# slatedb/slatedb

Hardware: AMD Instinct MI355X
Metric: GiB/s device-resident SST block encode+bloom, 64 MiB sorted KV, 1/2/4/8 GPU (higher is better)
Workload: dtype u8

## Files before the change

### slatedb_amd/csrc/sdb_encode.h

```cpp
#pragma once
#include <hip/hip_runtime.h>
#include <stdint.h>

#include "../../include/slatedb_amd.h"

namespace sdb {

constexpr uint32_t kChunk = 2048;
constexpr uint32_t kResolveLds = 96 * 1024;
#ifndef SDB_EMIT_CRC_MFMA
#define SDB_EMIT_CRC_SLICE
#endif
#ifdef SDB_EMIT_CRC_SLICE
constexpr uint32_t kCrcLds = 36 * 1024;
#else
constexpr uint32_t kCrcLds = 56 * 1024;
#endif
constexpr uint32_t kImgCap = 4096 + 64;
constexpr uint32_t kStageCap = 4096;
constexpr uint32_t kStageGuard = 64;
constexpr uint32_t kKeyStageCap = 1024;
constexpr uint32_t kPieceRowMax = 4000, kPieceKeyMax = 960, kPieceValMax = 3968;
constexpr uint32_t kSegLook = 1024;
constexpr uint32_t kSegSpan = kChunk + kSegLook;
// ... 58 lines not shown
    uint32_t *lcp;
    uint32_t *szr, *sznr;
    uint64_t *hd;
    uint32_t nfacts;
    uint32_t *row_scratch;
    uint32_t *next;
    uint32_t *bbytes;
    uint32_t *tab_exit;
    uint32_t *tab_cnt;
    uint64_t *tab_bytes;
    uint32_t *anchor_e;
    uint32_t *anchor_blk;
    uint64_t *anchor_byte;
    unsigned long long *err;
    uint32_t *wmax;
    uint32_t *slow_count;
    uint32_t *slow_list;
    uint32_t *big_count;
    uint32_t *big_list;
    BlockDesc *desc;
    uint64_t *stat_part;
    uint32_t *huge_part;
    uint32_t *wmax_part;
    unsigned long long *err_part;
    uint32_t *gtab_exit;
    uint32_t *gtab_cnt;
    uint64_t *gtab_bytes;
    uint32_t *mode;
    uint32_t group;
    uint32_t bloom_fused;
    BloomPlan bpl;
    BloomSlots bq;
    uint8_t *bloom_out;
    uint32_t *done;
    uint32_t nprep_wg;
    uint32_t seg_lds;
    uint8_t *out_data;
    uint64_t *out_block_off;
    uint32_t *out_block_first;
    uint32_t *out_index_key_len;
    uint16_t *out_block_stats;
    uint64_t data_cap, block_cap;
    sdb_sst_summary *summary;
    uint64_t bloom_len;
    uint32_t num_probes, filter_built;
    const uint64_t *bloom_len_dev;
};

struct EncodeWorkspace {
    uint64_t lcp, szr, sznr, hd, row_scratch, next, bbytes, tab_exit, tab_cnt, tab_bytes;
    uint64_t anchor_e, anchor_blk, anchor_byte, err, wmax, slow_count, slow_list, big_count, big_list, desc, stat_part,
        huge_part, wmax_part,
        bloom_rep;
    uint64_t err_part, done, gtab_exit, gtab_cnt, gtab_bytes, mode, blen;
    uint64_t total;
};
uint64_t bloom_workspace_bytes(uint64_t n, uint32_t k, uint64_t bitmap_bytes);
uint64_t encode_bloom_workspace_bytes(uint64_t n, uint32_t k, uint64_t bitmap_bytes);
__host__ __device__ inline EncodeWorkspace encode_workspace_offsets(uint64_t n, bool has_filter) {
    EncodeWorkspace w{};
    uint64_t off = 0;
    auto take = [&](uint64_t bytes) {
        uint64_t r = off;
        off += (bytes + 255) & ~255ull;
        return r;
    };
    uint64_t nc = (n + kChunk - 1) / kChunk;
    w.lcp = take(4 * (n + 1));
    w.szr = take(4 * (n + 1));
    w.sznr = take(4 * (n + 1));
    w.hd = take(0);
    (void)has_filter;
    w.row_scratch = take(4 * (n + 1));
    w.next = take(4 * (n + 1));
    w.bbytes = take(4 * (n + 1));
    w.tab_exit = take(4 * (nc * kSegLook + 1));
    w.tab_cnt = take(4 * (nc * kSegLook + 1));
    w.tab_bytes = take(8 * (nc * kSegLook + 1));
    w.anchor_e = take(4 * (nc + 2));
    w.anchor_blk = take(4 * (nc + 2));
    w.anchor_byte = take(8 * (nc + 2));
    w.err = take(8);
    w.wmax = take(4);
    w.slow_count = take(4);
    w.slow_list = take(4 * (n + 1));
    w.big_count = take(4);
    w.big_list = take(4 * (n + 1));
    w.desc = take(sizeof(BlockDesc) * (n + 1));
    const uint64_t nf = (n + kFactsEntries - 1) / kFactsEntries;
    w.stat_part = take(8 * 5 * (nf + 1));
    w.huge_part = take(4 * (nf + 1));
    w.wmax_part = take(4 * (nc + 1));
    w.err_part = take(8 * (nf + 1));
    w.done = take(8);
    w.gtab_exit = take(4 * (nc * kSegLook + 1));
    w.gtab_cnt = take(4 * (nc * kSegLook + 1));
    w.gtab_bytes = take(8 * (nc * kSegLook + 1));
    w.mode = take(4);
    w.blen = take(8);
    w.bloom_rep = off;
    w.total = off;
    return w;
}
inline EncodeWorkspace encode_workspace_layout(uint64_t n, uint64_t filter_bytes, uint32_t num_probes) {
    EncodeWorkspace w = encode_workspace_offsets(n, filter_bytes != 0);
    w.total = w.bloom_rep + ((filter_bytes ? encode_bloom_workspace_bytes(n, num_probes, filter_bytes) : 0) + 255) / 256 * 256;
    return w;
}
uint64_t prefix_workspace_bytes(uint64_t n);
hipError_t launch_bloom_prefix(const uint8_t *key_bytes, const uint64_t *key_off, const int32_t *lens, uint64_t n,
                               uint32_t bpk, uint32_t kind, uint32_t arg, uint32_t whole, uint8_t *bitmap, uint64_t cap,
                               uint64_t *bloom_len, void *ws, hipStream_t st);
hipError_t launch_bloom_match(const uint8_t *bitmap, uint64_t bytes, uint32_t k, uint32_t whole, uint32_t kind,
                              uint32_t arg, const uint8_t *key_bytes, const uint64_t *key_off, const uint8_t *is_prefix,
                              const int32_t *qlens, uint64_t n, uint8_t *result, hipStream_t st);

constexpr uint32_t kMaxSsts = 8;
enum WsField {
    kWsLcp = 0, kWsSzr, kWsSznr, kWsHd, kWsRowScratch, kWsNext, kWsBbytes, kWsTabExit, kWsTabCnt, kWsTabBytes,
    kWsAnchorE, kWsAnchorBlk, kWsAnchorByte, kWsErr, kWsWmax, kWsSlowCount, kWsSlowList, kWsBigCount, kWsBigList,
    kWsDesc, kWsStatPart, kWsHugePart, kWsWmaxPart, kWsBloomRep, kWsErrPart, kWsDone, kWsGtabExit, kWsGtabCnt,
    kWsGtabBytes, kWsMode, kWsBlen, kWsFields
};
struct SstSlot {
    const uint8_t *key_bytes;
    const uint64_t *key_off;
    const uint8_t *val_bytes;
    const uint64_t *val_off;
    const uint8_t *kind;
    const uint64_t *seq;
    const int64_t *create_ts;
    const int64_t *expire_ts;
    const uint8_t *ts_mask;
    uint64_t n;
    uint8_t *out_data;
    uint64_t *out_block_off;
    uint32_t *out_block_first;
    uint32_t *out_index_key_len;
    uint16_t *out_block_stats;
    uint64_t data_cap, block_cap;
    sdb_sst_summary *summary;
    uint8_t *bloom_out;
    uint64_t bloom_len;
    uint8_t *ws;
    uint32_t num_probes, filter_built, bloom_fused, has_filter_ws;
    uint32_t nchunks, nfacts, group, slot_cap;
    uint32_t prefix_bloom, pad2;
    BloomPlan bpl;
    uint32_t wso[kWsFields];
};
struct SstSet {
    uint32_t count;
    uint32_t block_size, restart_interval, version, wal, seg_look;
    uint32_t max_facts, max_chunks, max_groups, max_tiles, max_slices, pad;
    SstSlot s[kMaxSsts];
};

__host__ __device__ inline EncodeArgs make_args(const SstSet &P, uint32_t i) {
    const SstSlot &s = P.s[i];
    EncodeArgs a{};
    a.key_bytes = s.key_bytes;
    a.key_off = s.key_off;
    a.val_bytes = s.val_bytes;
    a.val_off = s.val_off;
    a.kind = s.kind;
    a.seq = s.seq;
    a.create_ts = s.create_ts;
    a.expire_ts = s.expire_ts;
    a.ts_mask = s.ts_mask;
    a.n = s.n;
    a.block_size = P.block_size;
    a.restart_interval = P.restart_interval;
    a.version = P.version;
    a.wal = P.wal;
    a.nchunks = s.nchunks;
    a.seg_look = P.seg_look;
    uint8_t *b = s.ws;
    auto W = [&](int f) { return b + ((uint64_t)s.wso[f] << 8); };
    a.lcp = (uint32_t *)W(kWsLcp);
    a.szr = (uint32_t *)W(kWsSzr);
    a.sznr = (uint32_t *)W(kWsSznr);
    a.hd = (uint64_t *)W(kWsHd);
    a.nfacts = s.nfacts;
    a.row_scratch = (uint32_t *)W(kWsRowScratch);
    a.next = (uint32_t *)W(kWsNext);
    a.bbytes = (uint32_t *)W(kWsBbytes);
    a.tab_exit = (uint32_t *)W(kWsTabExit);
    a.tab_cnt = (uint32_t *)W(kWsTabCnt);
    a.tab_bytes = (uint64_t *)W(kWsTabBytes);
    a.anchor_e = (uint32_t *)W(kWsAnchorE);
    a.anchor_blk = (uint32_t *)W(kWsAnchorBlk);
    a.anchor_byte = (uint64_t *)W(kWsAnchorByte);
    a.err = (unsigned long long *)W(kWsErr);
    a.wmax = (uint32_t *)W(kWsWmax);
    a.slow_count = (uint32_t *)W(kWsSlowCount);
    a.slow_list = (uint32_t *)W(kWsSlowList);
    a.big_count = (uint32_t *)W(kWsBigCount);
    a.big_list = (uint32_t *)W(kWsBigList);
    a.desc = (BlockDesc *)W(kWsDesc);
    a.stat_part = (uint64_t *)W(kWsStatPart);
    a.huge_part = (uint32_t *)W(kWsHugePart);
    a.wmax_part = (uint32_t *)W(kWsWmaxPart);
    a.err_part = (unsigned long long *)W(kWsErrPart);
    a.gtab_exit = (uint32_t *)W(kWsGtabExit);
    a.gtab_cnt = (uint32_t *)W(kWsGtabCnt);
    a.gtab_bytes = (uint64_t *)W(kWsGtabBytes);
    a.mode = (uint32_t *)W(kWsMode);
    a.group = s.group;
    a.bloom_fused = s.bloom_fused;
    a.bpl = s.bpl;
    {
        uint8_t *q = W(kWsBloomRep);
        a.bq.count = (uint32_t *)q;
        a.bq.slot = (uint32_t *)(q + (((uint64_t)s.bpl.tiles * s.bpl.nslices * 4 + 255) & ~255ull));
        a.bq.cap = s.slot_cap;
    }
    a.bloom_out = s.bloom_out;
    a.done = (uint32_t *)W(kWsDone);
    a.nprep_wg = s.nchunks;
    a.seg_lds = kSegLds;
    a.out_data = s.out_data;
    a.out_block_off = s.out_block_off;
    a.out_block_first = s.out_block_first;
    a.out_index_key_len = s.out_index_key_len;
    a.out_block_stats = s.out_block_stats;
    a.data_cap = s.data_cap;
    a.block_cap = s.block_cap;
    a.summary = s.summary;
    a.bloom_len = s.bloom_len;
    a.num_probes = s.num_probes;
    a.filter_built = s.filter_built;
    a.bloom_len_dev = s.prefix_bloom ? (uint64_t *)W(kWsBlen) : nullptr;
    return a;
}

inline void fill_ws_layout(SstSlot &s) {
    const EncodeWorkspace w = encode_workspace_offsets(s.n, s.has_filter_ws != 0);
    const uint64_t off[kWsFields] = {w.lcp, w.szr, w.sznr, w.hd, w.row_scratch, w.next, w.bbytes, w.tab_exit, w.tab_cnt,
                                     w.tab_bytes, w.anchor_e, w.anchor_blk, w.anchor_byte, w.err, w.wmax, w.slow_count,
                                     w.slow_list, w.big_count, w.big_list, w.desc, w.stat_part, w.huge_part, w.wmax_part,
                                     w.bloom_rep, w.err_part, w.done, w.gtab_exit, w.gtab_cnt, w.gtab_bytes, w.mode, w.blen};
    for (int f = 0; f < kWsFields; f++) s.wso[f] = (uint32_t)(off[f] >> 8);
}

hipError_t launch_encode_set(const SstSet &P, size_t bin_lds, size_t fill_lds, hipStream_t st);
hipError_t launch_encode_empty(EncodeArgs a, hipStream_t st);
hipError_t launch_encode_prep(const SstSet &P, hipStream_t st);

enum Stage { kStBloom = 0, kStFacts, kStSeg, kStAnchor, kStBlocks, kStEmit, kStEmitBig, kStBloomFill, kNumStages };
void stage_mark(hipStream_t st, int stage, bool begin);
bool stage_timing_on();


BloomPlan bloom_plan(uint64_t n, uint32_t k, uint64_t bitmap_bytes, uint32_t tile_keys = 0);
uint64_t bloom_workspace_bytes(uint64_t n, uint32_t k, uint64_t bitmap_bytes);
hipError_t launch_bloom_build(const uint8_t *key_bytes, const uint64_t *key_off, uint64_t n,
                              uint32_t num_probes, uint8_t *bitmap, uint64_t bitmap_bytes, void *ws,
                              hipStream_t st);
hipError_t launch_bloom_query(const uint8_t *bitmap, uint64_t bitmap_bytes, uint32_t num_probes,
                              const uint8_t *key_bytes, const uint64_t *key_off, uint64_t n,
                              uint8_t *result, hipStream_t st);

}
static_assert(sdb::kSegSpan % sdb::kSegThreads == 0 && sdb::kChunk % 64 == 0, "k_seg geometry");
static_assert(sdb::kEmitLds <= 160 * 1024, "k_emit LDS");
static_assert(sizeof(sdb::SstSet) <= 4096, "SstSet is passed as kernel arguments");
```

### slatedb_amd/csrc/sdb_encode.hip

```cpp
#include <stdlib.h>

#include <atomic>
#include <mutex>

#include "sdb_bloom.h"
#include "sdb_crc.h"
#include "sdb_crc_mfma.h"

namespace sdb {

#ifndef SDB_SEG_WAVES
#define SDB_SEG_WAVES 8
#endif
#ifdef SDB_PHASE_TIMING
__device__ uint64_t g_phase[1024][8];
#define PHASE_MARK(i)                                                              \
    do {                                                                           \
        __syncthreads();                                                           \
        if (threadIdx.x == 0 && blockIdx.x < 1024) g_phase[blockIdx.x][i] = __builtin_amdgcn_s_memtime(); \
    } while (0)
__device__ uint64_t g_wave_phase[8192][8];
__device__ uint64_t g_phase_enum[1024][8];
#define PHASE_MARK_E(i)                                                                  \
    do {                                                                                 \
        __syncthreads();                                                                 \
        if (threadIdx.x == 0 && blockIdx.x < 1024) g_phase_enum[blockIdx.x][i] = __builtin_amdgcn_s_memtime(); \
    } while (0)
__device__ uint64_t g_wave_rt[8192][4];
#define WAVE_T(var)                                     \
    uint64_t var = __builtin_amdgcn_s_memtime();        \
    __builtin_amdgcn_s_waitcnt(0xC07F)
#define PHASE_MARK_AT(slot, i)                                                        \
    do {                                                                          \
        __syncthreads();                                                          \
        if (threadIdx.x == 0) g_phase[slot][i] = __builtin_amdgcn_s_memtime();   \
    } while (0)
#else
#define PHASE_MARK(i) \
    do {              \
    } while (0)
#define PHASE_MARK_AT(slot, i) \
    do {                       \
    } while (0)
#define PHASE_MARK_E(i) \
    do {                \
    } while (0)
#define WAVE_T(var) \
    do {            \
    } while (0)
#endif


struct EntryFacts {
    uint32_t lcp, s_r, s_nr;
    uint64_t klen, vlen;
    uint8_t kind;
    int err;
};

struct FactsIn {
    uint64_t pko, ko0, ko1, vo0, vo1;
    uint64_t pk0, pk1, ck0, ck1;
    uint8_t kd, m;
};

SDB_DEV void facts_load_offsets(const EncodeArgs &a, uint64_t i, FactsIn &in) {
    in.ko0 = a.key_off[i];
    in.ko1 = a.key_off[i + 1];
    in.pko = i > 0 ? a.key_off[i - 1] : in.ko0;
    in.vo0 = a.val_off[i];
    in.vo1 = a.val_off[i + 1];
    in.kd = a.kind ? a.kind[i] : 0;
    in.m = a.ts_mask ? a.ts_mask[i] : 0;
}

SDB_DEV void facts_load_keys(const EncodeArgs &a, FactsIn &in) {
    const uint64_t klen = in.ko1 - in.ko0, plen = in.ko0 - in.pko;
    uint64_t n = klen < plen ? klen : plen;
    n = n < 16 ? n : 16;
    in.pk0 = in.ck0 = in.pk1 = in.ck1 = 0;
    if (n) {
        const uint32_t n0 = (uint32_t)(n < 8 ? n : 8);
        in.pk0 = load8(a.key_bytes + in.pko, n0);
        in.ck0 = load8(a.key_bytes + in.ko0, n0);
        if (n > 8) {
            in.pk1 = load8(a.key_bytes + in.pko + 8, (uint32_t)(n - 8));
            in.ck1 = load8(a.key_bytes + in.ko0 + 8, (uint32_t)(n - 8));
        }
    }
}

SDB_DEV EntryFacts facts_finish(const EncodeArgs &a, uint64_t i, const FactsIn &in) {
    EntryFacts f;
    const uint64_t klen = in.ko1 - in.ko0;
    const uint8_t kd = in.kd, m = in.m;
    const uint64_t vlen = (kd == SDB_KIND_TOMBSTONE) ? 0 : (in.vo1 - in.vo0);
    uint32_t lcp = 0;
    int err = 0;
    if (kd > SDB_KIND_TOMBSTONE) err = SDB_INVALID_ARGUMENT;
    if (!err && i > 0) {
        const uint64_t plen = in.ko0 - in.pko;
        const uint64_t mn = plen < klen ? plen : klen;
        const uint32_t nmin = (uint32_t)(mn > 0xFFFFFFFFull ? 0xFFFFFFFFull : mn);
        const uint32_t n0 = nmin < 8 ? nmin : 8, n1 = nmin < 16 ? nmin - n0 : 8;
        uint64_t x0 = in.pk0 ^ in.ck0, x1 = in.pk1 ^ in.ck1;
        if (n0 < 8) x0 &= (1ull << (8 * n0)) - 1;
        if (n1 < 8) x1 &= (1ull << (8 * n1)) - 1;
        if (x0) lcp = __builtin_ctzll(x0) >> 3;
        else if (x1) lcp = 8 + (__builtin_ctzll(x1) >> 3);
        else if (nmin <= 16) lcp = nmin;
        else lcp = 16 + lcp_bytes(a.key_bytes + in.pko + 16, nmin - 16, a.key_bytes + in.ko0 + 16, nmin - 16);
        if (klen == 0) err = SDB_EMPTY_KEY;
        else if (!a.wal && plen > 0 && lcp == klen && klen < plen) err = SDB_INVALID_ARGUMENT;
    }
    if (!err && klen == 0) err = SDB_EMPTY_KEY;
    const uint32_t ts8 = 8u * (((m & SDB_TS_CREATE) != 0) + ((m & SDB_TS_EXPIRE) != 0));
    if (a.version == 2) {
        if (!err && (klen > 0xFFFFFFFFull || vlen > 0xFFFFFFFFull)) err = SDB_LIMIT_EXCEEDED;
        uint32_t kl = (uint32_t)klen, vl = (uint32_t)vlen, suf = kl - lcp;
        f.s_nr = varint_len(lcp) + varint_len(suf) + varint_len(vl) + suf + vl + 9 + ts8;
        f.s_r = 1 + varint_len(kl) + varint_len(vl) + kl + vl + 9 + ts8;
    } else {
        if (!err && (klen > 0xFFFF || vlen > 0xFFFFFFFFull)) err = SDB_LIMIT_EXCEEDED;
        f.s_r = (uint32_t)(4 + klen + 9 + ts8 + (kd == SDB_KIND_TOMBSTONE ? 0 : 4 + vlen));
        f.s_nr = f.s_r;
    }
    f.lcp = lcp;
    f.klen = klen;
    f.vlen = vlen;
    f.kind = kd;
    f.err = err;
    return f;
}

SDB_DEV EntryFacts entry_facts(const EncodeArgs &a, uint64_t i) {
    FactsIn in;
    facts_load_offsets(a, i, in);
    facts_load_keys(a, in);
    return facts_finish(a, i, in);
}

__global__ __launch_bounds__(kFactsThreads, 8) void k_facts(SstSet P) {
    const EncodeArgs a = make_args(P, blockIdx.y);
    if (blockIdx.x >= a.nfacts) return;
    extern __shared__ __attribute__((aligned(16))) uint32_t blds[];
    __shared__ uint64_t s_part[kFactsThreads / 64][5];
    __shared__ unsigned long long s_err[kFactsThreads / 64];
    __shared__ uint32_t s_huge[kFactsThreads / 64];
    const uint32_t tid = threadIdx.x, lane = (uint32_t)lane_id();
    const uint64_t e0 = (uint64_t)blockIdx.x * kFactsEntries + tid;
    const uint64_t n = a.n;
    FactsIn in[kFactsPerT];
#pragma unroll
    for (uint32_t r = 0; r < kFactsPerT; r++) {
        const uint64_t e = e0 + r * kFactsThreads;
        FactsIn &f = in[r];
        f.ko0 = f.ko1 = f.vo0 = f.vo1 = f.pko = 0;
        f.kd = f.m = 0;
        if (e <= n) {
            f.ko0 = a.key_off[e];
            f.vo0 = a.val_off[e];
            if (e < n) {
                f.kd = a.kind ? a.kind[e] : 0;
                f.m = a.ts_mask ? a.ts_mask[e] : 0;
                if (lane == 63) {
                    f.ko1 = a.key_off[e + 1];
                    f.vo1 = a.val_off[e + 1];
                }
                if (lane == 0 && e > 0) f.pko = a.key_off[e - 1];
            }
        }
    }
    const uint64_t ktot = a.key_off[n];
#pragma unroll
    for (uint32_t r = 0; r < kFactsPerT; r++) {
        FactsIn &f = in[r];
        const uint64_t nk = wave_next_lane(f.ko0), nv = wave_next_lane(f.vo0);
        if (lane != 63) {
            f.ko1 = nk;
            f.vo1 = nv;
        }
        const uint64_t e = e0 + r * kFactsThreads;
        const bool live = e < n;
        const uint8_t *safe = (const uint8_t *)a.key_off;
        const uint8_t *cs = live && f.ko0 + 16 <= ktot ? a.key_bytes + f.ko0 : safe;
        uint4 cw;
        __builtin_memcpy(&cw, cs, 16);
        f.ck0 = (uint64_t)cw.x | (uint64_t)cw.y << 32;
        f.ck1 = (uint64_t)cw.z | (uint64_t)cw.w << 32;
        f.pk0 = f.pk1 = 0;
    }
#pragma unroll
    for (uint32_t r = 0; r < kFactsPerT; r++) {
        FactsIn &f = in[r];
        const uint64_t e = e0 + r * kFactsThreads;
        if (lane == 0 && e > 0 && e < n && f.pko + 16 <= ktot) {
            uint4 pw;
            __builtin_memcpy(&pw, a.key_bytes + f.pko, 16);
            f.pk0 = (uint64_t)pw.x | (uint64_t)pw.y << 32;
            f.pk1 = (uint64_t)pw.z | (uint64_t)pw.w << 32;
        }
    }
#pragma unroll
    for (uint32_t r = 0; r < kFactsPerT; r++) {
        FactsIn &f = in[r];
        const uint64_t e = e0 + r * kFactsThreads;
        if (e < n && f.ko0 + 16 > ktot) {
            const uint64_t kl = f.ko1 - f.ko0;
            const uint32_t kn = (uint32_t)(kl < 16 ? kl : 16);
            f.ck0 = f.ck1 = 0;
            if (kn) f.ck0 = load8(a.key_bytes + f.ko0, kn < 8 ? kn : 8);
            if (kn > 8) f.ck1 = load8(a.key_bytes + f.ko0 + 8, kn - 8);
        }
        if (lane == 0 && e > 0 && e < n && f.pko + 16 > ktot) {
            const uint64_t pl = f.ko0 - f.pko;
            const uint32_t pn = (uint32_t)(pl < 16 ? pl : 16);
            f.pk0 = f.pk1 = 0;
            if (pn) f.pk0 = load8(a.key_bytes + f.pko, pn < 8 ? pn : 8);
            if (pn > 8) f.pk1 = load8(a.key_bytes + f.pko + 8, pn - 8);
        }
    }
    uint64_t rk = 0, rv = 0, c = 0;
    uint64_t err = ~0ull;
    bool huge = false;
    uint32_t hh[kFactsPerT], dd[kFactsPerT];
#pragma unroll
    for (uint32_t r = 0; r < kFactsPerT; r++) {
        FactsIn &f = in[r];
        const uint64_t e = e0 + r * kFactsThreads;
        {
            const uint64_t pko = wave_prev_lane(f.ko0), pk0 = wave_prev_lane(f.ck0), pk1 = wave_prev_lane(f.ck1);
            if (lane != 0) {
                f.pko = pko;
                f.pk0 = pk0;
                f.pk1 = pk1;
            } else if (e == 0) {
                f.pko = f.ko0;
            }
        }
        hh[r] = dd[r] = 0;
        if (e < n) {
            const EntryFacts x = facts_finish(a, e, f);
            a.lcp[e] = x.lcp;
            a.szr[e] = x.s_r;
            a.sznr[e] = x.s_nr;
            if (a.bloom_fused) {
                const uint64_t kl = f.ko1 - f.ko0;
#ifdef SDB_EXP_FACTS_NOHASH
                const uint64_t h = (f.ck0 * 0x9E3779B97F4A7C15ull) ^ (f.ck1 + kl);
#else
                const uint64_t h = kl == 16 ? siphash13_16(f.ck0, f.ck1) : siphash13(a.key_bytes + f.ko0, kl);
#endif
                hh[r] = fastmod_u32((uint32_t)h, a.bpl.mmod, a.bpl.m);
                dd[r] = fastmod_u32((uint32_t)(h >> 32), a.bpl.mmod, a.bpl.m);
            }
            if (x.err) {
                const uint64_t ev = (e << 8) | (uint64_t)x.err;
                err = ev < err ? ev : err;
            }
            huge |= x.s_r > kPieceRowMax || x.klen > kPieceKeyMax || x.vlen > kPieceValMax;
            rk += x.klen;
            rv += x.vlen;
            c += (uint64_t)(x.kind == SDB_KIND_VALUE) | ((uint64_t)(x.kind == SDB_KIND_TOMBSTONE) << 20) |
                 ((uint64_t)(x.kind == SDB_KIND_MERGE) << 40);
        }
    }
    rk = wave_sum(rk);
    rv = wave_sum(rv);
    c = wave_sum(c);
    err = wave_readlane(wave_incl_scan_op(err, [](uint64_t x, uint64_t y) { return x < y ? x : y; }), 63);
    const uint32_t w = tid >> 6;
    if (lane == 0) {
        s_part[w][0] = rk;
        s_part[w][1] = rv;
        s_part[w][2] = c & 0xFFFFF;
        s_part[w][3] = (c >> 20) & 0xFFFFF;
        s_part[w][4] = (c >> 40) & 0xFFFFF;
        s_err[w] = err;
    }
    const bool wh = __ballot(huge) != 0;
    if (lane == 0) s_huge[w] = wh ? 1u : 0u;
    __syncthreads();
    if (tid < 5) {
        uint64_t t = 0;
        for (uint32_t q = 0; q < kFactsThreads / 64; q++) t += s_part[q][tid];
        a.stat_part[5 * (uint64_t)blockIdx.x + tid] = t;
    }
    if (tid == 0) {
        unsigned long long m = ~0ull;
        for (uint32_t q = 0; q < kFactsThreads / 64; q++) m = s_err[q] < m ? s_err[q] : m;
        a.err_part[blockIdx.x] = m;
        uint32_t h = 0;
        for (uint32_t q = 0; q < kFactsThreads / 64; q++) h |= s_huge[q];
        a.huge_part[blockIdx.x] = h;
    }
    if (a.bloom_fused) {
        const uint64_t k0 = (uint64_t)blockIdx.x * kFactsEntries;
        const uint32_t nk = (uint32_t)((k0 + kFactsEntries < n ? k0 + kFactsEntries : n) - k0);
#ifdef SDB_EXP_FACTS_NOBIN
        bloom_bin_core<kFactsPerT>(blockIdx.x, hh, dd, 0, a.bpl, a.bq, blds);
#else
        bloom_bin_core<kFactsPerT>(blockIdx.x, hh, dd, nk, a.bpl, a.bq, blds);
#endif
    }
}

SDB_DEV uint32_t walk_size_v2(const EncodeArgs &a, uint64_t j, bool rs) {
    EntryFacts f = entry_facts(a, j);
    return rs ? f.s_r : f.s_nr;
}

SDB_DEV void seg_chunk(const EncodeArgs &a, uint8_t *smem, uint32_t k) {
    uint32_t *s_P = (uint32_t *)smem;
    uint32_t *s_R = s_P + kSegSpan + 4;
    uint32_t *s_bb = s_R + kSegSpan;
    uint16_t *s_nx = (uint16_t *)(s_bb + kChunk);
    __shared__ uint32_t s_len[kSegThreads / 64];
    const uint32_t tid = threadIdx.x, nt = blockDim.x;
    const uint64_t cs = (uint64_t)k * kChunk;
    const uint64_t ce = cs + kChunk < a.n ? cs + kChunk : a.n;
    const uint64_t se = ce + a.seg_look < a.n ? ce + a.seg_look : a.n;
    const uint32_t cn = (uint32_t)(ce - cs), sn = (uint32_t)(se - cs);
    const uint64_t bs = a.block_size;
    const uint32_t clampv = (uint32_t)(bs + 16);
    const bool v2 = a.version == 2 && bs <= (1u << 20);
    const uint32_t ri = a.restart_interval;
    PHASE_MARK(0);
    constexpr uint32_t kPerT = kSegSpan / kSegThreads;
    const uint32_t lane = (uint32_t)lane_id();
    uint32_t zr[kPerT], znr[kPerT];
#pragma unroll
    for (uint32_t u = 0; u < kPerT; u++) {
        const uint32_t x = tid + u * nt;
        zr[u] = znr[u] = 0;
        if (x < sn) {
            zr[u] = a.szr[cs + x];
            znr[u] = a.sznr[cs + x];
        }
    }
#pragma unroll
    for (uint32_t u = 0; u < kPerT; u++) {
        const uint32_t x = tid + u * nt;
        if (x >= sn) continue;
        if (v2) {
            const uint32_t cr = zr[u] < clampv ? zr[u] : clampv, cnr = znr[u] < clampv ? znr[u] : clampv;
            s_P[x] = cnr;
            s_R[x] = cr + 2 - cnr;
        }
    }
    __syncthreads();
    PHASE_MARK(1);
    if (v2) {
        __shared__ uint32_t s_wt[kPerT * (kSegThreads / 64) + 1];
        const uint32_t wv = tid >> 6;
        uint32_t v[kPerT], inc[kPerT];
#pragma unroll
        for (uint32_t u = 0; u < kPerT; u++) {
            const uint32_t x = tid + u * nt;
            v[u] = x < sn ? s_P[x] : 0;
            inc[u] = wave_incl_scan(v[u]);
            if (lane == 63) s_wt[u * (nt >> 6) + wv] = inc[u];
        }
        __syncthreads();
        if (tid < 64) {
            const uint32_t nw = kPerT * (nt >> 6);
            const uint32_t t = tid < nw ? s_wt[tid] : 0, it = wave_incl_scan(t);
            __builtin_amdgcn_wave_barrier();
            if (tid < nw) s_wt[tid] = it - t;
            if (tid == 63) s_P[sn] = it;
        }
        __syncthreads();
#pragma unroll
        for (uint32_t u = 0; u < kPerT; u++) {
            const uint32_t x = tid + u * nt;
            if (x < sn) s_P[x] = s_wt[u * (nt >> 6) + wv] + inc[u] - v[u];
        }
        PHASE_MARK(2);
    }
    __syncthreads();
    PHASE_MARK(3);
    uint32_t maxlen = 0;
    for (uint32_t x = tid; x < cn; x += nt) {
        const uint64_t b = cs + x;
        uint64_t j;
        uint64_t bytes;
        if (v2) {
            const uint32_t Pb = s_P[x];
            auto size_of = [&](uint32_t e) -> uint64_t {
                uint64_t sz = 2ull + (s_P[e] - Pb);
                for (uint32_t r = x; r < e; r += ri) sz += s_R[r];
                return sz;
            };
            uint32_t lo = x + 1;
            uint32_t e = lo;
            {
                const uint32_t w = (x + 64 < sn ? x + 64 : sn) - x;
                const uint32_t mean = (s_P[x + w] - Pb) / w + 1;
                uint32_t est = x + (uint32_t)(bs / mean);
                e = est < lo ? lo : (est > sn ? sn : est);
            }
            if (size_of(e) <= bs) {
                while (e < sn && size_of(e + 1) <= bs) e++;
            } else {
                while (e > lo && size_of(e) > bs) e--;
            }
            j = cs + e;
            if (e == lo) bytes = 2ull + a.szr[b] + 2;
            else bytes = size_of(e);
            if (e == sn && se < a.n) {
                uint64_t acc = bytes;
                uint32_t p = e - x, ph = p % ri;
                while (j < a.n) {
                    const bool rs = ph == 0;
                    const uint64_t add = (uint64_t)walk_size_v2(a, j, rs) + (rs ? 2 : 0);
                    if (acc + add > bs) break;
                    acc += add;
                    j++;
                    if (++ph == ri) ph = 0;
                }
                bytes = acc;
            }
        } else if (a.version == 2) {
            uint64_t acc = 2;
            j = b;
            uint32_t p = 0, ph = 0;
            while (j < a.n) {
                const bool rs = ph == 0;
                const uint64_t add = (uint64_t)walk_size_v2(a, j, rs) + (rs ? 2 : 0);
                if (p > 0 && acc + add > bs) break;
                acc += add;
                j++;
                p++;
                if (++ph == ri) ph = 0;
            }
            bytes = acc;
        } else {
            uint64_t acc = 2;
            j = b;
            uint32_t p = 0;
            const uint64_t fko = a.key_off[b];
            const uint32_t fkl = (uint32_t)(a.key_off[b + 1] - fko);
            while (j < a.n) {
                uint32_t prefix = 0;
                if (p > 0) {
                    uint64_t ko = a.key_off[j];
                    prefix = lcp_bytes(a.key_bytes + fko, fkl, a.key_bytes + ko, (uint32_t)(a.key_off[j + 1] - ko));
                }
                uint64_t sr = a.szr[j];
                uint64_t sz = sr - prefix;
                if (p > 0 && acc + sz > bs) break;
                acc += sz + 2;
                j++;
                p++;
            }
            bytes = acc;
        }
        const uint32_t bb = (uint32_t)(bytes + 4);
// ... 2052 lines not shown
    }
}

template __global__ void k_emit<1>(SstSet);
template __global__ void k_emit<2>(SstSet);

template <int V>
__global__ __launch_bounds__(kEmitThreads, 1) void k_emit_big(SstSet P) {
    extern __shared__ __attribute__((aligned(16))) uint8_t smem[];
    uint32_t pre[kMaxSsts + 1];
    pre[0] = 0;
#pragma unroll
    for (uint32_t i = 0; i < kMaxSsts; i++) {
        uint32_t nb = 0;
        if (i < P.count) {
            const EncodeArgs ai = make_args(P, i);
            if (*ai.err == ~0ull) nb = *ai.big_count;
        }
        pre[i + 1] = pre[i] + nb;
    }
    const uint32_t total = pre[kMaxSsts];
    if (!total || lds_addr((const void *)smem) != 0) return;
    crc_tables_to_lds((lu32 *)smem);
    __syncthreads();
    const uint32_t wave = (uint32_t)__builtin_amdgcn_readfirstlane((int)(threadIdx.x >> 6)), wpb = blockDim.x >> 6;
    lu8 *img = (lu8 *)smem + kCrcLds + 16 + wave * kEmitWaveLds + kStageGuard;
    lu8 *kst = img + kImgCap + 16;
    lSpanCopy *rtab = (lSpanCopy *)(kst + kKeyStageCap);
    for (uint32_t g = blockIdx.x * wpb + wave; g < total; g += gridDim.x * wpb) {
        uint32_t si = 0, base = 0;
#pragma unroll
        for (uint32_t j = 1; j < kMaxSsts; j++)
            if (g >= pre[j] && pre[j] < total) {
                si = j;
                base = pre[j];
            }
        const EncodeArgs a = make_args(P, si);
        const uint32_t blk = a.big_list[g - base];
        emit_big<V>(a, blk, a.desc[blk], img, kst, rtab);
    }
}
template __global__ void k_emit_big<1>(SstSet);
template __global__ void k_emit_big<2>(SstSet);

__global__ void k_init_summary(EncodeArgs a) {
    if (threadIdx.x == 0) {
        sdb_sst_summary *s = a.summary;
        s->data_len = 0;
        s->num_blocks = 0;
        s->num_entries = a.n;
        s->raw_key_size = 0;
        s->raw_val_size = 0;
        s->num_puts = s->num_deletes = s->num_merges = 0;
        s->bloom_len = 0;
        s->num_probes = 0;
        s->filter_built = 0;
        s->status = 0;
        s->max_block_entries = 0;
        s->first_error_entry = ~0ull;
        *a.err = ~0ull;
        *a.wmax = 0;
        *a.slow_count = 0;
        *a.big_count = 0;
        if (a.n == 0 && a.block_cap + 1 > 0) {
            a.out_block_off[0] = 0;
            a.out_block_first[0] = 0;
        }
    }
}

__global__ void k_finish_summary(EncodeArgs a, uint64_t bloom_len, uint32_t num_probes, uint32_t built) {
    if (threadIdx.x == 0) {
        sdb_sst_summary *s = a.summary;
        unsigned long long e = *a.err;
        s->max_block_entries = *a.wmax;
        s->bloom_len = bloom_len;
        s->num_probes = num_probes;
        s->filter_built = built;
        if (e != ~0ull) {
            s->status = (int32_t)(e & 0xFF);
            s->first_error_entry = e >> 8;
        }
    }
}

#ifdef SDB_PHASE_TIMING
extern "C" int sdb_diag_wave_phase(uint64_t *out, int nwaves) {
    return hipMemcpyFromSymbol(out, HIP_SYMBOL(g_wave_phase), sizeof(uint64_t) * 8 * nwaves) == hipSuccess ? 0 : -1;
}
extern "C" int sdb_diag_wave_rt(uint64_t *out, int nwaves) {
#ifdef SDB_PHASE_TIMING
    return hipMemcpyFromSymbol(out, HIP_SYMBOL(g_wave_rt), sizeof(uint64_t) * 4 * nwaves) == hipSuccess ? 0 : -1;
#else
    return -1;
#endif
}
extern "C" int sdb_diag_enum_phase(uint64_t *out, int nblocks) {
    return hipMemcpyFromSymbol(out, HIP_SYMBOL(g_phase_enum), sizeof(uint64_t) * 8 * nblocks) == hipSuccess ? 0 : -1;
}
extern "C" int sdb_diag_phase_times(uint64_t *out, int nblocks) {
    return hipMemcpyFromSymbol(out, HIP_SYMBOL(g_phase), sizeof(uint64_t) * 8 * nblocks) == hipSuccess ? 0 : -1;
}
#endif

static int g_cus = 0;
static uint32_t g_emit_threads = kEmitThreads, g_emit_wg_per_cu = kEmitWgPerCu;
static std::once_flag g_attrs_once;
static uint32_t g_emit_grid = 0;
constexpr int kMaxDevices = 64;
static std::atomic<uint32_t> g_builders[kMaxDevices];
static int current_device() {
    int dev = 0;
    return hipGetDevice(&dev) == hipSuccess && dev >= 0 && dev < kMaxDevices ? dev : 0;
}
static uint32_t emit_grid() {
    if (g_emit_grid) return g_emit_grid;
    const uint32_t full = (uint32_t)(g_cus > 0 ? g_emit_wg_per_cu * g_cus : 512);
    const uint32_t b = g_builders[current_device()].load(std::memory_order_relaxed);
    return b > 1 ? (full / b ? full / b : 1u) : full;
}
static uint32_t emit_lds() { return kCrcLds + 16 + (g_emit_threads / 64) * kEmitWaveLds; }
static void set_lds_attrs() {
    std::call_once(g_attrs_once, [] {
        int dev = 0;
        (void)hipGetDevice(&dev);
        (void)hipDeviceGetAttribute(&g_cus, hipDeviceAttributeMultiprocessorCount, dev);
        if (const char *e = getenv("SDB_EMIT_THREADS")) {
            uint32_t t = (uint32_t)atoi(e);
            if (t >= 64 && t <= kEmitThreads && t % 64 == 0) g_emit_threads = t;
        }
        if (const char *e = getenv("SDB_EMIT_GRID")) {
            const int t = atoi(e);
            if (t >= 1 && t <= 4096) g_emit_grid = (uint32_t)t;
        }
        if (const char *e = getenv("SDB_EMIT_WG_PER_CU")) {
            uint32_t t = (uint32_t)atoi(e);
            if (t >= 1 && t <= 32) g_emit_wg_per_cu = t;
        }
        (void)hipFuncSetAttribute((const void *)k_emit<1>, hipFuncAttributeMaxDynamicSharedMemorySize, (int)kEmitLds);
        (void)hipFuncSetAttribute((const void *)k_emit<2>, hipFuncAttributeMaxDynamicSharedMemorySize, (int)kEmitLds);
        (void)hipFuncSetAttribute((const void *)k_emit_big<1>, hipFuncAttributeMaxDynamicSharedMemorySize, (int)kEmitLds);
        (void)hipFuncSetAttribute((const void *)k_emit_big<2>, hipFuncAttributeMaxDynamicSharedMemorySize, (int)kEmitLds);
        (void)hipFuncSetAttribute((const void *)k_enum, hipFuncAttributeMaxDynamicSharedMemorySize, (int)kEnumLds);
        (void)hipFuncSetAttribute((const void *)k_group, hipFuncAttributeMaxDynamicSharedMemorySize, (int)kGroupLds);
        (void)hipFuncSetAttribute((const void *)k_anchor, hipFuncAttributeMaxDynamicSharedMemorySize, (int)kAnchorLds);
        (void)hipFuncSetAttribute((const void *)k_seg, hipFuncAttributeMaxDynamicSharedMemorySize, 96 * 1024);
        (void)hipFuncSetAttribute((const void *)k_facts, hipFuncAttributeMaxDynamicSharedMemorySize, (int)kBinLds);
        (void)hipGetLastError();
    });
}

static_assert(kChunk == kFactsEntries && kFactsThreads == kBinThreads, "bloom tiles are k_facts' chunks of kChunk keys");

hipError_t launch_encode_set(const SstSet &P, size_t bin_lds, size_t fill_lds, hipStream_t st) {
    set_lds_attrs();
    if (!P.count) return hipSuccess;
    stage_mark(st, kStFacts, true);
    hipLaunchKernelGGL(k_facts, dim3(P.max_facts, P.count), dim3(kFactsThreads), P.max_tiles ? bin_lds : 0, st, P);
    stage_mark(st, kStFacts, false);
    stage_mark(st, kStSeg, true);
    const size_t seg_lds = kSegLds > fill_lds ? kSegLds : fill_lds;
    hipLaunchKernelGGL(k_seg, dim3(P.max_chunks + P.max_slices, P.count), dim3(kSegThreads), seg_lds, st, P);
    stage_mark(st, kStSeg, false);
    stage_mark(st, kStAnchor, true);
    hipLaunchKernelGGL(k_anchor, dim3(1, P.count), dim3(kAnchorThreads), kAnchorLds, st, P);
    stage_mark(st, kStAnchor, false);
    stage_mark(st, kStBlocks, true);
    hipLaunchKernelGGL(k_blocks, dim3(P.max_chunks, P.count), dim3(kBlkThreads), 0, st, P);
    stage_mark(st, kStBlocks, false);
    stage_mark(st, kStEmitBig, true);
    const uint32_t big_grid = P.block_size > 4096 ? emit_grid() : (emit_grid() < 32 ? emit_grid() : 32);
    if (P.version == 2) hipLaunchKernelGGL(k_emit_big<2>, dim3(big_grid), dim3(g_emit_threads), emit_lds(), st, P);
    else hipLaunchKernelGGL(k_emit_big<1>, dim3(big_grid), dim3(g_emit_threads), emit_lds(), st, P);
    stage_mark(st, kStEmitBig, false);
    stage_mark(st, kStEmit, true);
    if (P.version == 2) hipLaunchKernelGGL(k_emit<2>, dim3(emit_grid()), dim3(g_emit_threads), emit_lds(), st, P);
    else hipLaunchKernelGGL(k_emit<1>, dim3(emit_grid()), dim3(g_emit_threads), emit_lds(), st, P);
    stage_mark(st, kStEmit, false);
    return hipGetLastError();
}

hipError_t launch_encode_prep(const SstSet &P, hipStream_t st) {
    set_lds_attrs();
    if (!P.count) return hipSuccess;
    hipLaunchKernelGGL(k_facts, dim3(P.max_facts, P.count), dim3(kFactsThreads), 0, st, P);
    hipLaunchKernelGGL(k_seg, dim3(P.max_chunks, P.count), dim3(kSegThreads), kSegLds, st, P);
    hipLaunchKernelGGL(k_group, dim3(P.max_groups, P.count), dim3(kGroupThreads), kGroupLds, st, P);
    return hipGetLastError();
}

hipError_t launch_encode_empty(EncodeArgs a, hipStream_t st) {
    hipLaunchKernelGGL(k_init_summary, dim3(1), dim3(64), 0, st, a);
    hipLaunchKernelGGL(k_finish_summary, dim3(1), dim3(64), 0, st, a, a.bloom_len, a.num_probes, a.filter_built);
    return hipGetLastError();
}

}

extern "C" sdb_status sdb_set_concurrent_builders(uint32_t builders) {
    if (builders == 0) return SDB_INVALID_ARGUMENT;
    sdb::g_builders[sdb::current_device()].store(builders, std::memory_order_relaxed);
    return SDB_OK;
}
```

Before: 1228.

## Add 32-bit narrow-offset fast path to k_facts tiles

Adds a narrow path in k_facts that, when the key and value byte spans fit in 32 bits, loads only the low halves of the offsets and does all per-entry arithmetic and reductions in 32-bit. It also shares neighbour offsets and the first 16 key bytes across lanes with wave shuffles instead of loading them again from memory. The aim is less ALU, register and load work in the facts stage, with the shared per-tile epilogue moved into a helper. In exchange it keeps two code paths and adds per-block range checks, and the kind-count packing now uses 10-bit fields, which assumes per-wave counts stay below 1024.

```diff
diff --git a/slatedb_amd/csrc/sdb_encode.h b/slatedb_amd/csrc/sdb_encode.h
--- a/slatedb_amd/csrc/sdb_encode.h
+++ b/slatedb_amd/csrc/sdb_encode.h
@@ -234,7 +234,8 @@
 struct SstSet {
     uint32_t count;
     uint32_t block_size, restart_interval, version, wal, seg_look;
-    uint32_t max_facts, max_chunks, max_groups, max_tiles, max_slices, pad;
+    uint32_t max_facts, max_chunks, max_groups, max_tiles, max_slices;
+    uint32_t facts_narrow_limit;
     SstSlot s[kMaxSsts];
 };
 
diff --git a/slatedb_amd/csrc/sdb_encode.hip b/slatedb_amd/csrc/sdb_encode.hip
--- a/slatedb_amd/csrc/sdb_encode.hip
+++ b/slatedb_amd/csrc/sdb_encode.hip
@@ -140,13 +140,293 @@
     return facts_finish(a, i, in);
 }
 
+struct FactsLds {
+    uint64_t part[kFactsThreads / 64][5];
+    unsigned long long err[kFactsThreads / 64];
+    uint32_t huge[kFactsThreads / 64];
+};
+
+SDB_DEV void facts_tile_finish(const EncodeArgs &a, FactsLds &s, const uint32_t (&hh)[kFactsPerT],
+                               const uint32_t (&dd)[kFactsPerT], uint32_t *blds) {
+    const uint32_t tid = threadIdx.x;
+    const uint64_t n = a.n;
+    __syncthreads();
+    if (tid < 5) {
+        uint64_t t = 0;
+        for (uint32_t q = 0; q < kFactsThreads / 64; q++) t += s.part[q][tid];
+        a.stat_part[5 * (uint64_t)blockIdx.x + tid] = t;
+    }
+    if (tid == 0) {
+        unsigned long long m = ~0ull;
+        for (uint32_t q = 0; q < kFactsThreads / 64; q++) m = s.err[q] < m ? s.err[q] : m;
+        a.err_part[blockIdx.x] = m;
+        uint32_t h = 0;
+        for (uint32_t q = 0; q < kFactsThreads / 64; q++) h |= s.huge[q];
+        a.huge_part[blockIdx.x] = h;
+    }
+    if (a.bloom_fused) {
+        const uint64_t k0 = (uint64_t)blockIdx.x * kFactsEntries;
+        const uint32_t nk = (uint32_t)((k0 + kFactsEntries < n ? k0 + kFactsEntries : n) - k0);
+#ifdef SDB_EXP_FACTS_NOBIN
+        bloom_bin_core<kFactsPerT>(blockIdx.x, hh, dd, 0, a.bpl, a.bq, blds);
+#else
+        bloom_bin_core<kFactsPerT>(blockIdx.x, hh, dd, nk, a.bpl, a.bq, blds);
+#endif
+    }
+}
+
+struct FactsIn32 {
+    uint32_t pko, ko0, ko1, vo0, vo1;
+    uint32_t pk[4], ck[4];
+    uint8_t kd, m;
+};
+struct EntryFacts32 {
+    uint32_t lcp, s_r, s_nr, klen, vlen;
+    uint8_t kind;
+    int err;
+};
+
+SDB_DEV EntryFacts32 facts_finish32(const EncodeArgs &a, bool has_prev, const uint8_t *kbase, const FactsIn32 &in) {
+    EntryFacts32 f;
+    const uint32_t klen = in.ko1 - in.ko0;
+    const uint8_t kd = in.kd, m = in.m;
+    const uint32_t vlen = (kd == SDB_KIND_TOMBSTONE) ? 0 : (in.vo1 - in.vo0);
+    uint32_t lcp = 0;
+    int err = 0;
+    if (kd > SDB_KIND_TOMBSTONE) err = SDB_INVALID_ARGUMENT;
+    if (!err && has_prev) {
+        const uint32_t plen = in.ko0 - in.pko;
+        const uint32_t nmin = plen < klen ? plen : klen;
+        const uint64_t x0 = ((uint64_t)(in.pk[1] ^ in.ck[1]) << 32) | (in.pk[0] ^ in.ck[0]);
+        const uint64_t x1 = ((uint64_t)(in.pk[3] ^ in.ck[3]) << 32) | (in.pk[2] ^ in.ck[2]);
+        const uint32_t d = x0 ? (uint32_t)(__builtin_ctzll(x0) >> 3) : x1 ? 8 + (uint32_t)(__builtin_ctzll(x1) >> 3) : 16;
+        if (d < 16 || nmin <= 16) lcp = d < nmin ? d : nmin;
+        else lcp = 16 + lcp_bytes(kbase + in.pko + 16, nmin - 16, kbase + in.ko0 + 16, nmin - 16);
+        if (klen == 0) err = SDB_EMPTY_KEY;
+        else if (!a.wal && plen > 0 && lcp == klen && klen < plen) err = SDB_INVALID_ARGUMENT;
+    }
+    if (!err && klen == 0) err = SDB_EMPTY_KEY;
+    const uint32_t ts8 = 8u * (((m & SDB_TS_CREATE) != 0) + ((m & SDB_TS_EXPIRE) != 0));
+    if (a.version == 2) {
+        const uint32_t suf = klen - lcp;
+        f.s_nr = varint_len(lcp) + varint_len(suf) + varint_len(vlen) + suf + vlen + 9 + ts8;
+        f.s_r = 1 + varint_len(klen) + varint_len(vlen) + klen + vlen + 9 + ts8;
+    } else {
+        if (!err && klen > 0xFFFF) err = SDB_LIMIT_EXCEEDED;
+        f.s_r = 4 + klen + 9 + ts8 + (kd == SDB_KIND_TOMBSTONE ? 0 : 4 + vlen);
+        f.s_nr = f.s_r;
+    }
+    f.lcp = lcp;
+    f.klen = klen;
+    f.vlen = vlen;
+    f.kind = kd;
+    f.err = err;
+    return f;
+}
+
+SDB_DEV uint32_t facts_nrel(const EncodeArgs &a, uint64_t t0) {
+    return (uint32_t)(a.n - t0 < kFactsEntries + 1 ? a.n - t0 : kFactsEntries + 1);
+}
+
+SDB_DEV void facts_narrow_load(const EncodeArgs &a, uint64_t t0, FactsIn32 (&in)[kFactsPerT]) {
+    const uint32_t tid = threadIdx.x, lane = (uint32_t)lane_id();
+    const uint32_t nrel = facts_nrel(a, t0);
+    const bool tile0 = t0 == 0;
+    const uint32_t *kol = (const uint32_t *)(a.key_off + t0), *vol = (const uint32_t *)(a.val_off + t0);
+    const uint8_t *kindb = a.kind ? a.kind + t0 : nullptr, *maskb = a.ts_mask ? a.ts_mask + t0 : nullptr;
+#pragma unroll
+    for (uint32_t r = 0; r < kFactsPerT; r++) {
+        const uint32_t i = tid + r * kFactsThreads;
+        FactsIn32 &f = in[r];
+        f.ko0 = f.ko1 = f.vo0 = f.vo1 = f.pko = 0;
+        f.kd = f.m = 0;
+        if (i <= nrel) {
+            f.ko0 = kol[2 * i];
+            f.vo0 = vol[2 * i];
+            if (i < nrel) {
+                f.kd = kindb ? kindb[i] : 0;
+                f.m = maskb ? maskb[i] : 0;
+                if (lane == 63) {
+                    f.ko1 = kol[2 * i + 2];
+                    f.vo1 = vol[2 * i + 2];
+                }
+                if (lane == 0 && (i > 0 || !tile0)) f.pko = kol[2 * (int32_t)i - 2];
+            }
+        }
+    }
+}
+
+SDB_DEV void facts_tile_narrow(const EncodeArgs &a, uint64_t t0, FactsLds &s, uint32_t (&hh)[kFactsPerT],
+                                  uint32_t (&dd)[kFactsPerT]) {
+    const uint32_t tid = threadIdx.x, lane = (uint32_t)lane_id();
+    const uint32_t nrel = facts_nrel(a, t0);
+    const bool tile0 = t0 == 0;
+    const uint64_t kb = a.key_off[t0 ? t0 - 1 : 0], vb = a.val_off[t0];
+    const uint8_t *kbase = a.key_bytes + kb;
+    const uint32_t kb32 = (uint32_t)kb, vb32 = (uint32_t)vb;
+    FactsIn32 in[kFactsPerT];
+    facts_narrow_load(a, t0, in);
+#pragma unroll
+    for (uint32_t r = 0; r < kFactsPerT; r++) {
+        FactsIn32 &f = in[r];
+        f.ko0 -= kb32;
+        f.ko1 -= kb32;
+        f.pko -= kb32;
+        f.vo0 -= vb32;
+        f.vo1 -= vb32;
+    }
+    const uint64_t ktr = a.key_off[a.n] - kb;
+    const bool anyk = ktr >= 16;
+    const uint32_t klim = (uint32_t)(ktr > 0xFFFFFFFFull ? 0xFFFFFFFFull : ktr) - 16;
+    const uint8_t *wbase = anyk ? kbase : (const uint8_t *)a.key_off;
+#pragma unroll
+    for (uint32_t r = 0; r < kFactsPerT; r++) {
+        FactsIn32 &f = in[r];
+        const uint32_t nk = wave_next_lane(f.ko0), nv = wave_next_lane(f.vo0);
+        if (lane != 63) {
+            f.ko1 = nk;
+            f.vo1 = nv;
+        }
+        const uint32_t i = tid + r * kFactsThreads;
+        const uint32_t wo = i < nrel && anyk && f.ko0 <= klim ? f.ko0 : 0;
+        uint4 cw;
+        __builtin_memcpy(&cw, wbase + wo, 16);
+        f.ck[0] = cw.x;
+        f.ck[1] = cw.y;
+        f.ck[2] = cw.z;
+        f.ck[3] = cw.w;
+        f.pk[0] = f.pk[1] = f.pk[2] = f.pk[3] = 0;
+    }
+#pragma unroll
+    for (uint32_t r = 0; r < kFactsPerT; r++) {
+        FactsIn32 &f = in[r];
+        const uint32_t i = tid + r * kFactsThreads;
+        if (lane == 0 && (i > 0 || !tile0) && i < nrel && anyk && f.pko <= klim) {
+            uint4 pw;
+            __builtin_memcpy(&pw, kbase + f.pko, 16);
+            f.pk[0] = pw.x;
+            f.pk[1] = pw.y;
+            f.pk[2] = pw.z;
+            f.pk[3] = pw.w;
+        }
+    }
+#pragma unroll
+    for (uint32_t r = 0; r < kFactsPerT; r++) {
+        FactsIn32 &f = in[r];
+        const uint32_t i = tid + r * kFactsThreads;
+        if (i < nrel && !(anyk && f.ko0 <= klim)) {
+            const uint32_t kl = f.ko1 - f.ko0;
+            const uint32_t kn = kl < 16 ? kl : 16;
+            uint64_t c0 = 0, c1 = 0;
+            if (kn) c0 = load8(kbase + f.ko0, kn < 8 ? kn : 8);
+            if (kn > 8) c1 = load8(kbase + f.ko0 + 8, kn - 8);
+            f.ck[0] = (uint32_t)c0;
+            f.ck[1] = (uint32_t)(c0 >> 32);
+            f.ck[2] = (uint32_t)c1;
+            f.ck[3] = (uint32_t)(c1 >> 32);
+        }
+        if (lane == 0 && (i > 0 || !tile0) && i < nrel && !(anyk && f.pko <= klim)) {
+            const uint32_t pl = f.ko0 - f.pko;
+            const uint32_t pn = pl < 16 ? pl : 16;
+            uint64_t p0 = 0, p1 = 0;
+            if (pn) p0 = load8(kbase + f.pko, pn < 8 ? pn : 8);
+            if (pn > 8) p1 = load8(kbase + f.pko + 8, pn - 8);
+            f.pk[0] = (uint32_t)p0;
+            f.pk[1] = (uint32_t)(p0 >> 32);
+            f.pk[2] = (uint32_t)p1;
+            f.pk[3] = (uint32_t)(p1 >> 32);
+        }
+    }
+    uint32_t rk = 0, rv = 0, c = 0, nerr = 0;
+    bool huge = false;
+    uint32_t *lcpo = a.lcp + t0, *szro = a.szr + t0, *sznro = a.sznr + t0;
+#pragma unroll
+    for (uint32_t r = 0; r < kFactsPerT; r++) {
+        FactsIn32 &f = in[r];
+        const uint32_t i = tid + r * kFactsThreads;
+        {
+            const uint32_t pko = wave_prev_lane(f.ko0);
+            const uint32_t p0 = wave_prev_lane(f.ck[0]), p1 = wave_prev_lane(f.ck[1]);
+            const uint32_t p2 = wave_prev_lane(f.ck[2]), p3 = wave_prev_lane(f.ck[3]);
+            if (lane != 0) {
+                f.pko = pko;
+                f.pk[0] = p0;
+                f.pk[1] = p1;
+                f.pk[2] = p2;
+                f.pk[3] = p3;
+            } else if (i == 0 && tile0) {
+                f.pko = f.ko0;
+            }
+        }
+        hh[r] = dd[r] = 0;
+        if (i < nrel) {
+            const EntryFacts32 x = facts_finish32(a, i > 0 || !tile0, kbase, f);
+            lcpo[i] = x.lcp;
+            szro[i] = x.s_r;
+            sznro[i] = x.s_nr;
+            if (a.bloom_fused) {
+                const uint64_t ck0 = ((uint64_t)f.ck[1] << 32) | f.ck[0], ck1 = ((uint64_t)f.ck[3] << 32) | f.ck[2];
+#ifdef SDB_EXP_FACTS_NOHASH
+                const uint64_t h = (ck0 * 0x9E3779B97F4A7C15ull) ^ (ck1 + x.klen);
+#else
+                const uint64_t h = x.klen == 16 ? siphash13_16(ck0, ck1) : siphash13(kbase + f.ko0, x.klen);
+#endif
+                hh[r] = fastmod_u32((uint32_t)h, a.bpl.mmod, a.bpl.m);
+                dd[r] = fastmod_u32((uint32_t)(h >> 32), a.bpl.mmod, a.bpl.m);
+            }
+            if (x.err) {
+                const uint32_t ne = ~((i << 8) | (uint32_t)x.err);
+                nerr = ne > nerr ? ne : nerr;
+            }
+            huge |= x.s_r > kPieceRowMax || x.klen > kPieceKeyMax || x.vlen > kPieceValMax;
+            rk += x.klen;
+            rv += x.vlen;
+            c += (uint32_t)(x.kind == SDB_KIND_VALUE) | ((uint32_t)(x.kind == SDB_KIND_TOMBSTONE) << 10) |
+                 ((uint32_t)(x.kind == SDB_KIND_MERGE) << 20);
+        }
+    }
+    rk = wave_sum(rk);
+    rv = wave_sum(rv);
+    c = wave_sum(c);
+    nerr = wave_max(nerr);
+    const uint32_t w = tid >> 6;
+    if (lane == 0) {
+        s.part[w][0] = rk;
+        s.part[w][1] = rv;
+        s.part[w][2] = c & 0x3FF;
+        s.part[w][3] = (c >> 10) & 0x3FF;
+        s.part[w][4] = (c >> 20) & 0x3FF;
+        s.err[w] = nerr ? (t0 << 8) + (uint32_t)~nerr : ~0ull;
+    }
+    const bool wh = __ballot(huge) != 0;
+    if (lane == 0) s.huge[w] = wh ? 1u : 0u;
+}
+
 __global__ __launch_bounds__(kFactsThreads, 8) void k_facts(SstSet P) {
     const EncodeArgs a = make_args(P, blockIdx.y);
     if (blockIdx.x >= a.nfacts) return;
     extern __shared__ __attribute__((aligned(16))) uint32_t blds[];
-    __shared__ uint64_t s_part[kFactsThreads / 64][5];
-    __shared__ unsigned long long s_err[kFactsThreads / 64];
-    __shared__ uint32_t s_huge[kFactsThreads / 64];
+    __shared__ FactsLds s;
+    {
+        const uint64_t t0 = (uint64_t)blockIdx.x * kFactsEntries;
+        const uint64_t lim = P.facts_narrow_limit ? P.facts_narrow_limit : 1ull << 32;
+        const uint64_t kfirst = a.key_off[0], klast = a.key_off[a.n], vfirst = a.val_off[0], vlast = a.val_off[a.n];
+        bool narrow = (klast - kfirst < lim) & (vlast - vfirst < lim);
+        if (!narrow) {
+            const uint64_t t1 = t0 + kFactsEntries < a.n ? t0 + kFactsEntries : a.n;
+            const uint64_t kb = a.key_off[t0 ? t0 - 1 : 0], vb = a.val_off[t0];
+            narrow = (a.key_off[t1] - kb < lim) & (a.val_off[t1] - vb < lim);
+        }
+        if (narrow) {
+            uint32_t sst = blockIdx.y;
+            asm volatile("" : "+s"(sst));
+            uint32_t hh[kFactsPerT], dd[kFactsPerT];
+            facts_tile_narrow(make_args(P, sst), t0, s, hh, dd);
+            asm volatile("" : "+s"(sst));
+            facts_tile_finish(make_args(P, sst), s, hh, dd, blds);
+            return;
+        }
+    }
     const uint32_t tid = threadIdx.x, lane = (uint32_t)lane_id();
     const uint64_t e0 = (uint64_t)blockIdx.x * kFactsEntries + tid;
     const uint64_t n = a.n;
@@ -271,38 +551,16 @@
     err = wave_readlane(wave_incl_scan_op(err, [](uint64_t x, uint64_t y) { return x < y ? x : y; }), 63);
     const uint32_t w = tid >> 6;
     if (lane == 0) {
-        s_part[w][0] = rk;
-        s_part[w][1] = rv;
-        s_part[w][2] = c & 0xFFFFF;
-        s_part[w][3] = (c >> 20) & 0xFFFFF;
-        s_part[w][4] = (c >> 40) & 0xFFFFF;
-        s_err[w] = err;
+        s.part[w][0] = rk;
+        s.part[w][1] = rv;
+        s.part[w][2] = c & 0xFFFFF;
+        s.part[w][3] = (c >> 20) & 0xFFFFF;
+        s.part[w][4] = (c >> 40) & 0xFFFFF;
+        s.err[w] = err;
     }
     const bool wh = __ballot(huge) != 0;
-    if (lane == 0) s_huge[w] = wh ? 1u : 0u;
-    __syncthreads();
-    if (tid < 5) {
-        uint64_t t = 0;
-        for (uint32_t q = 0; q < kFactsThreads / 64; q++) t += s_part[q][tid];
-        a.stat_part[5 * (uint64_t)blockIdx.x + tid] = t;
-    }
-    if (tid == 0) {
-        unsigned long long m = ~0ull;
-        for (uint32_t q = 0; q < kFactsThreads / 64; q++) m = s_err[q] < m ? s_err[q] : m;
-        a.err_part[blockIdx.x] = m;
-        uint32_t h = 0;
-        for (uint32_t q = 0; q < kFactsThreads / 64; q++) h |= s_huge[q];
-        a.huge_part[blockIdx.x] = h;
-    }
-    if (a.bloom_fused) {
-        const uint64_t k0 = (uint64_t)blockIdx.x * kFactsEntries;
-        const uint32_t nk = (uint32_t)((k0 + kFactsEntries < n ? k0 + kFactsEntries : n) - k0);
-#ifdef SDB_EXP_FACTS_NOBIN
-        bloom_bin_core<kFactsPerT>(blockIdx.x, hh, dd, 0, a.bpl, a.bq, blds);
-#else
-        bloom_bin_core<kFactsPerT>(blockIdx.x, hh, dd, nk, a.bpl, a.bq, blds);
-#endif
-    }
+    if (lane == 0) s.huge[w] = wh ? 1u : 0u;
+    facts_tile_finish(a, s, hh, dd, blds);
 }
 
 SDB_DEV uint32_t walk_size_v2(const EncodeArgs &a, uint64_t j, bool rs) {
@@ -2661,11 +2919,19 @@
 
 static_assert(kChunk == kFactsEntries && kFactsThreads == kBinThreads, "bloom tiles are k_facts' chunks of kChunk keys");
 
+static std::atomic<uint32_t> g_facts_narrow_limit{0};
+static SstSet with_facts_limit(const SstSet &P) {
+    SstSet Q = P;
+    Q.facts_narrow_limit = g_facts_narrow_limit.load(std::memory_order_relaxed);
+    return Q;
+}
+
 hipError_t launch_encode_set(const SstSet &P, size_t bin_lds, size_t fill_lds, hipStream_t st) {
     set_lds_attrs();
     if (!P.count) return hipSuccess;
     stage_mark(st, kStFacts, true);
-    hipLaunchKernelGGL(k_facts, dim3(P.max_facts, P.count), dim3(kFactsThreads), P.max_tiles ? bin_lds : 0, st, P);
+    hipLaunchKernelGGL(k_facts, dim3(P.max_facts, P.count), dim3(kFactsThreads), P.max_tiles ? bin_lds : 0, st,
+                       with_facts_limit(P));
     stage_mark(st, kStFacts, false);
     stage_mark(st, kStSeg, true);
     const size_t seg_lds = kSegLds > fill_lds ? kSegLds : fill_lds;
@@ -2692,7 +2958,7 @@
 hipError_t launch_encode_prep(const SstSet &P, hipStream_t st) {
     set_lds_attrs();
     if (!P.count) return hipSuccess;
-    hipLaunchKernelGGL(k_facts, dim3(P.max_facts, P.count), dim3(kFactsThreads), 0, st, P);
+    hipLaunchKernelGGL(k_facts, dim3(P.max_facts, P.count), dim3(kFactsThreads), 0, st, with_facts_limit(P));
     hipLaunchKernelGGL(k_seg, dim3(P.max_chunks, P.count), dim3(kSegThreads), kSegLds, st, P);
     hipLaunchKernelGGL(k_group, dim3(P.max_groups, P.count), dim3(kGroupThreads), kGroupLds, st, P);
     return hipGetLastError();
@@ -2706,6 +2972,10 @@
 
 }
 
+extern "C" void sdb_diag_facts_narrow_limit(uint64_t bytes) {
+    sdb::g_facts_narrow_limit.store(bytes >> 32 ? 0u : (uint32_t)bytes, std::memory_order_relaxed);
+}
+
 extern "C" sdb_status sdb_set_concurrent_builders(uint32_t builders) {
     if (builders == 0) return SDB_INVALID_ARGUMENT;
     sdb::g_builders[sdb::current_device()].store(builders, std::memory_order_relaxed);
```

Result: no change. 1232, median of 6 (+0.3%).
